# Visual-AI/SCD

Hardware: AMD Instinct MI355X
Metric: images/sec end-to-end (encode+sim+k-means) on 224^2 synth, 21k vocab (higher is better)
Workload: dtype f16; 1 GPU; ImageNet-100 unsupervised (BASELINE configs[1]): CLIP ViT-B/16 encode + V=21000 vocab + SSKM k=100 (10 restarts x 10 iters) + vote loop; cluster=SSKM, images_per_gpu=126976, vocab=21000, n_cluster=100, encode_batch=3990, weights=random-init (seeded), no checkpoint offline, parallelism=dp1

## Files before the change

### include/scd_hip.h

```cpp
#ifndef SCD_HIP_H
#define SCD_HIP_H
#include <stddef.h>
#include <stdint.h>

#ifdef __cplusplus
extern "C" {
#endif

typedef struct scd_ctx* scd_handle;
typedef struct scd_encoder scd_encoder;

enum scd_status { SCD_OK = 0, SCD_EINVAL = -1, SCD_EHIP = -2, SCD_ERCCL = -3, SCD_EINFEASIBLE = -4 };
enum scd_dtype { SCD_F32 = 0, SCD_F16 = 1 };
enum scd_sim_mode { SCD_SIM_RAW = 0, SCD_SIM_SOFTMAX = 1 };

int scd_version(void);
const char* scd_last_error(void);
int scd_create(int device, scd_handle* out);
int scd_destroy(scd_handle h);
int scd_trace_mark(scd_handle h, int end, void* stream);

int scd_l2norm_rows(scd_handle h, const void* x, int dtype, int64_t n, int d, void* out, void* stream);

size_t scd_sim_topk_ws_bytes(int64_t n, int d, int64_t v, int k);
// ... 175 lines not shown
int scd_comm_unique_id(void* id_out);
int scd_comm_init(scd_handle h, int rank, int world, const void* unique_id);
int scd_comm_destroy(scd_handle h);
int scd_allreduce_centroids(scd_handle h, double* packed, int64_t count, void* stream);
int scd_allgather_text(scd_handle h, const void* w_shard, int64_t shard_elems, void* w_full, void* stream);

typedef struct scd_encoder_desc {
    int kind;
    int width, layers, heads, mlp_dim;
    int tokens;
    int patch, image;
    int vocab;
    int out_dim;
    int act;
    float ln_eps;
    int registers;
} scd_encoder_desc;
int scd_encoder_create(scd_handle h, const scd_encoder_desc* desc, const void* const* weights, int n_weights,
                       scd_encoder** out);
int scd_encoder_destroy(scd_encoder* e);
size_t scd_encoder_ws_bytes(const scd_encoder* e, int batch);
int scd_encoder_timing(scd_encoder* e, int enable, double* ms_out, int* launches_out, double* flop_out);
int scd_vit_encode_image(scd_handle h, const scd_encoder* e, const void* pixels, int dtype, int batch, void* out,
                         int normalize, void* ws, size_t ws_bytes, void* stream);
int scd_clip_encode_text(scd_handle h, const scd_encoder* e, const int32_t* tokens, int batch, void* out,
                         int normalize, void* ws, size_t ws_bytes, void* stream);
int scd_clip_encode_text_len(scd_handle h, const scd_encoder* e, const int32_t* tokens, int batch, int ctx_len, void* out,
                             int normalize, void* ws, size_t ws_bytes, void* stream);
int scd_attention_f16(scd_handle h, const void* qkv, int batch, int T, int width, int heads, int causal, void* out, void* stream);
int scd_vit_assemble_f16(scd_handle h, const void* patch, const float* patch_bias, const float* cls, const float* pos,
                         const float* registers, int nreg, int batch, int T, int width, void* out, int64_t* stats, void* stream);
int scd_attention_single_query_f16(scd_handle h, const void* kv, const void* q, const int* qrow, int batch, int T, int width,
                                   int heads, int causal, void* out, void* stream);
int scd_gemm_f16(scd_handle h, const void* A, const void* W, const float* bias, const void* residual, void* C,
                 int64_t m, int n, int k, int act, void* stream);
int scd_gemm_ln_apply_f16(scd_handle h, const void* A, const void* Wf, const float* biasf, const float* colsum, const int64_t* stats_in,
                          float* rs, int64_t* zero_out, void* C, int64_t m, int n, int k, float eps, int act, void* stream);
int scd_gemm_res_stats_f16(scd_handle h, const void* A, const void* W, const float* bias, const void* residual, void* C,
                           int64_t* stats_out, int64_t m, int n, int k, int act, void* stream);
int scd_fold_ln_f16(scd_handle h, const void* W, const float* gamma, const float* beta, const float* bias, int n, int k, void* Wf,
                    float* colsum, float* biasf, void* stream);
int scd_gemm_img_f16(scd_handle h, const void* pixels, const void* W, void* C, int64_t m, int n, int batch, int image, void* stream);
int scd_layernorm_f16(scd_handle h, const void* x, const int* row_index, int64_t rows, int width, float eps, const float* gamma,
                      const float* beta, void* out, void* stream);

typedef struct scd_image_desc {
    int64_t src_off;
    int64_t tmp_off;
    int32_t w, h;
    int32_t plan_x;
    int32_t plan_y;
    int32_t row0, rows;
} scd_image_desc;
int scd_image_geometry(int w, int h, int size, int crop, int32_t* out6);
int scd_image_plan_axis(int in_size, int out_size, int off, int n, int32_t* first, int32_t* ntaps, int32_t* taps, int64_t taps_cap,
                        int64_t* n_taps_out);
int scd_image_batch_plan(const int32_t* wh, int batch, int size, int crop, scd_image_desc* descs, int32_t* plan, int64_t plan_cap,
                         int64_t* plan_len, int64_t* pixel_bytes, int64_t* ws_bytes);
int scd_image_preprocess(scd_handle h, const uint8_t* pixels, int64_t pixel_bytes, const scd_image_desc* descs, const int32_t* plan,
                         int64_t plan_len, int batch, int crop, const void* lut, void* out, void* ws, size_t ws_bytes, void* stream);

enum { SCD_JPEG_OK = 0, SCD_JPEG_NOT_JPEG = 1, SCD_JPEG_TRUNCATED = 2, SCD_JPEG_BAD_MARKER = 3, SCD_JPEG_PROGRESSIVE = 4, SCD_JPEG_ARITHMETIC = 5,
       SCD_JPEG_SOF = 6, SCD_JPEG_PRECISION = 7, SCD_JPEG_COMPONENTS = 8, SCD_JPEG_SAMPLING = 9, SCD_JPEG_COLOURSPACE = 10,
       SCD_JPEG_MULTISCAN = 11, SCD_JPEG_MISSING_TABLE = 12, SCD_JPEG_BAD_TABLE = 13, SCD_JPEG_CHROMA_WIDTH = 14, SCD_JPEG_DNL = 15 };
enum { SCD_JPEG_EHUFF = 1, SCD_JPEG_EINDEX = 2, SCD_JPEG_EEOF = 3, SCD_JPEG_EMARKER = 4, SCD_JPEG_ERANGE = 5, SCD_JPEG_EDESC = 6 };
typedef struct scd_jpeg_info {
// ... 33 lines not shown
```

### scd_amd/_lib.py

```python
import ctypes as C
import os
import threading

_HERE = os.path.dirname(os.path.abspath(__file__))
_LIB_PATH = os.environ.get("SCD_HIP_LIB") or os.path.join(_HERE, "lib", "libscd_hip.so")

SCD_OK, SCD_EINVAL, SCD_EHIP, SCD_ERCCL, SCD_EINFEASIBLE = 0, -1, -2, -3, -4
SCD_F32, SCD_F16 = 0, 1
SIM_RAW, SIM_SOFTMAX = 0, 1


class ScdError(RuntimeError):
    def __init__(self, code, msg):
        super().__init__("libscd_hip: %s (status %d)" % (msg, code))
        self.code = code


class EncoderDesc(C.Structure):
    _fields_ = [("kind", C.c_int), ("width", C.c_int), ("layers", C.c_int), ("heads", C.c_int), ("mlp_dim", C.c_int),
                ("tokens", C.c_int), ("patch", C.c_int), ("image", C.c_int), ("vocab", C.c_int), ("out_dim", C.c_int),
                ("act", C.c_int), ("ln_eps", C.c_float), ("registers", C.c_int)]


_vp, _i, _i64, _sz, _f = C.c_void_p, C.c_int, C.c_int64, C.c_size_t, C.c_float
# ... 87 lines not shown
    "scd_link_components_ws_bytes": (_sz, [_i64]),
    "scd_link_components": (_i, [_vp, _i64, _vp, _vp, _i64, _vp, _vp, _vp, _sz, _vp]),
    "scd_segment_mean_unit": (_i, [_vp, _vp, _i64, _vp, _vp, _i, _i, _vp, _vp, _vp]),
    "scd_knn_ws_bytes": (_sz, [_i64, _i64, _i, _i]),
    "scd_knn_slots": (_i, []),
    "scd_knn": (_i, [_vp, _vp, _i64, _vp, _i64, _i, _i, _i64, _vp, _vp, _vp, _vp, _sz, _vp]),
    "scd_knn_vote": (_i, [_vp, _vp, _vp, _i64, _i, _i, _vp, _i64, _i, C.c_double, _vp, _vp, _vp]),
    "scd_munkres": (_i, [_vp, _i, _i, _vp, C.POINTER(_i)]),
    "scd_munkres_sparse": (_i, [_i, _i64, _vp, _vp, _vp, _vp, C.POINTER(_i)]),
    "scd_transport_solve": (_i, [_vp, _i64, _i, _i, _i, _vp, C.POINTER(_i64)]),
    "scd_transport_solve_batch": (_i, [_vp, _i64, _i, _i, _i, _i, _vp, _vp, _i]),
    "scd_comm_unique_id_bytes": (_sz, []),
    "scd_comm_unique_id": (_i, [_vp]),
    "scd_comm_init": (_i, [_vp, _i, _i, _vp]),
    "scd_comm_destroy": (_i, [_vp]),
    "scd_allreduce_centroids": (_i, [_vp, _vp, _i64, _vp]),
    "scd_allgather_text": (_i, [_vp, _vp, _i64, _vp, _vp]),
    "scd_encoder_create": (_i, [_vp, C.POINTER(EncoderDesc), C.POINTER(_vp), _i, C.POINTER(_vp)]),
    "scd_encoder_destroy": (_i, [_vp]),
    "scd_encoder_ws_bytes": (_sz, [_vp, _i]),
    "scd_encoder_timing": (_i, [_vp, _i, C.POINTER(C.c_double), C.POINTER(_i), C.POINTER(C.c_double)]),
    "scd_vit_encode_image": (_i, [_vp, _vp, _vp, _i, _i, _vp, _i, _vp, _sz, _vp]),
    "scd_clip_encode_text": (_i, [_vp, _vp, _vp, _i, _vp, _i, _vp, _sz, _vp]),
    "scd_clip_encode_text_len": (_i, [_vp, _vp, _vp, _i, _i, _vp, _i, _vp, _sz, _vp]),
    "scd_gemm_f16": (_i, [_vp, _vp, _vp, _vp, _vp, _vp, _i64, _i, _i, _i, _vp]),
    "scd_gemm_ln_apply_f16": (_i, [_vp, _vp, _vp, _vp, _vp, _vp, _vp, _vp, _vp, _i64, _i, _i, _f, _i, _vp]),
    "scd_gemm_res_stats_f16": (_i, [_vp, _vp, _vp, _vp, _vp, _vp, _vp, _i64, _i, _i, _i, _vp]),
    "scd_fold_ln_f16": (_i, [_vp, _vp, _vp, _vp, _vp, _i, _i, _vp, _vp, _vp, _vp]),
    "scd_gemm_img_f16": (_i, [_vp, _vp, _vp, _vp, _i64, _i, _i, _i, _vp]),
    "scd_layernorm_f16": (_i, [_vp, _vp, _vp, _i64, _i, _f, _vp, _vp, _vp, _vp]),
    "scd_attention_f16": (_i, [_vp, _vp, _i, _i, _i, _i, _i, _vp, _vp]),
    "scd_vit_assemble_f16": (_i, [_vp, _vp, _vp, _vp, _vp, _vp, _i, _i, _i, _i, _vp, _vp, _vp]),
    "scd_attention_single_query_f16": (_i, [_vp, _vp, _vp, _vp, _i, _i, _i, _i, _i, _vp, _vp]),
    "scd_image_geometry": (_i, [_i, _i, _i, _i, _vp]),
    "scd_image_plan_axis": (_i, [_i, _i, _i, _i, _vp, _vp, _vp, _i64, _vp]),
    "scd_image_batch_plan": (_i, [_vp, _i, _i, _i, _vp, _vp, _i64, _vp, _vp, _vp]),
    "scd_image_preprocess": (_i, [_vp, _vp, _i64, _vp, _vp, _i64, _i, _i, _vp, _vp, _vp, _sz, _vp]),
    "scd_jpeg_parse": (_i, [_vp, _i64, _vp, _vp, _i64]),
    "scd_jpeg_batch_plan": (_i, [_vp, _vp, _vp, _i, _vp, _vp, _i64, _vp, _vp, _vp]),
    "scd_jpeg_decode": (_i, [_vp, _vp, _i64, _vp, _vp, _i64, _i, _vp, _i64, _vp, _vp, _sz, _vp]),
    "scd_jpeg_decode_host": (_i, [_vp, _i64, _vp, _i64, _vp]),
}

IMAGE_DESC_FIELDS = [("src_off", "<i8"), ("tmp_off", "<i8"), ("w", "<i4"), ("h", "<i4"), ("plan_x", "<i4"), ("plan_y", "<i4"),
                     ("row0", "<i4"), ("rows", "<i4")]

JPEG_INFO_FIELDS = [(k, "<i4") for k in ("reason", "w", "h", "ncomp", "hs", "vs", "restart_interval", "file_len", "scan_off", "scan_end",
                                          "has_eoi", "n_restarts")] + [(k, "<i4", (3,)) for k in ("qt_off", "qt_prec", "dc_off", "ac_off")]
JPEG_DESC_FIELDS = [("data_off", "<i8"), ("out_off", "<i8"), ("plane_off", "<i8")] + \
                   [(k, "<i4") for k in ("data_len", "scan_off", "scan_end", "has_eoi", "w", "h", "ncomp", "hs", "vs", "restart_interval")] + \
                   [(k, "<i4", (3,)) for k in ("qt", "dc", "ac")] + [("pad_", "<i4")]

_lock = threading.Lock()
_lib = None


def lib_path():
    return _LIB_PATH


def load():
    global _lib
    with _lock:
        if _lib is not None:
            return _lib
        if not os.path.exists(_LIB_PATH):
# ... 66 lines not shown
```

### scd_amd/csrc/encoder.hip

```cpp
#include "common.h"
#include "gemm.h"
#include <vector>
#include <stdlib.h>

struct scd_encoder {
    scd_encoder_desc d;
    std::vector<const void*> w;
    bool timing = false;
    std::vector<std::pair<hipEvent_t, hipEvent_t>> ev;
    double timed_flop = 0.0;
    struct Folded { const half_t *wq, *w1; const float *csq, *bq, *cs1, *b1; };
    std::vector<Folded> folded;
    void* folded_mem = nullptr;
    int kp = 0;
    half_t* wpatch_pad = nullptr;
};

enum { W_PATCH = 0, W_PATCH_B = 1, W_CLS = 2, W_POS = 3, W_LNPRE_W = 4, W_LNPRE_B = 5, W_LNPOST_W = 6, W_LNPOST_B = 7,
       W_PROJ = 8, W_LAYER0 = 9, W_PER_LAYER = 12 };
static inline int w_registers(const scd_encoder_desc& d) { return W_LAYER0 + W_PER_LAYER * d.layers; }
enum { L_LN1_W = 0, L_LN1_B, L_QKV_W, L_QKV_B, L_PROJ_W, L_PROJ_B, L_LN2_W, L_LN2_B, L_FC1_W, L_FC1_B, L_FC2_W, L_FC2_B };

__device__ __forceinline__ void stats_acc(const half4& o, float* st1, float* st2) {
#pragma unroll
    for (int j = 0; j < 4; ++j) {
        const float f = (float)o[j];
        *st1 += f;
        *st2 = fmaf(f, f, *st2);
    }
}
__device__ __forceinline__ void stats_store(float s1, float s2, long long* stats, long long r, int lane) {
    s1 = wave_sum_f32(s1);
    s2 = wave_sum_f32(s2);
    if (lane == 0) {
        stats[2 * r] = __float2ll_rn(s1 * 16777216.f);
        stats[2 * r + 1] = __float2ll_rn(s2 * 1048576.f);
    }
}
template <int MAXG>
__device__ __forceinline__ void ln_row(const float (&v)[MAXG][4], int groups, int width, float eps, const float* g,
                                       const float* b, half_t* out, int lane, float* st1 = nullptr, float* st2 = nullptr) {
    float s = 0.f;
#pragma unroll
    for (int i = 0; i < MAXG; ++i)
        if (i < groups) s += v[i][0] + v[i][1] + v[i][2] + v[i][3];
    const float mean = wave_sum_f32(s) / (float)width;
    float q = 0.f;
#pragma unroll
    for (int i = 0; i < MAXG; ++i)
// ... 854 lines not shown
#pragma unroll
    for (int e = 0; e < 8; ++e) o8[e] = 0.f;
    for (int key = ks; key < nkeys; key += 8) {
        const half8 v8 = *(const half8*)(vbase + (size_t)key * ldk + 8 * dc);
        const float pk = ps[wv][key];
#pragma unroll
        for (int e = 0; e < 8; ++e) o8[e] = fmaf(pk, (float)v8[e], o8[e]);
    }
    half8 o;
#pragma unroll
    for (int e = 0; e < 8; ++e) {
        float v = o8[e];
        v += __shfl_xor(v, 8, 64);
        v += __shfl_xor(v, 16, 64);
        v += __shfl_xor(v, 32, 64);
        o[e] = (half_t)(v * inv);
    }
    if (ks == 0) *(half8*)(out + (size_t)img * width + head * 64 + 8 * dc) = o;
}

__global__ void __launch_bounds__(256) gather2_rows_kernel(const half_t* __restrict__ a, const half_t* __restrict__ b,
                                                           const int* __restrict__ rows, int n, int width,
                                                           half_t* __restrict__ dst_a, half_t* __restrict__ dst_b) {
    const int lane = threadIdx.x & 63;
    const int i = blockIdx.x * 4 + (threadIdx.x >> 6);
    if (i >= n) return;
    const size_t src = (size_t)rows[i] * width, dst = (size_t)i * width;
    for (int c = lane * 8; c < width; c += 512) {
        *(half8*)(dst_a + dst + c) = *(const half8*)(a + src + c);
        *(half8*)(dst_b + dst + c) = *(const half8*)(b + src + c);
    }
}

struct EncPad {
    int batch, bh;
    int tokens;
    long long rows, prows;
};
static inline EncPad make_pad(const scd_encoder_desc& d, int batch, int tokens = 0) {
    EncPad p;
    p.batch = batch;
    p.tokens = tokens > 0 ? tokens : d.tokens;
    p.bh = (batch + 255) / 256 * 256;
    p.rows = ((long long)batch * p.tokens + 255) / 256 * 256;
    p.prows = ((long long)batch * (p.tokens - 1 - d.registers) + 255) / 256 * 256;
    return p;
}

struct EncWs {
    half_t *x, *y, *qkv, *h, *cls, *outp;
    int* rows;
    long long *stats_a, *stats_b;
    half_t *xsel, *ysel, *hsel;
    long long* stats_sel;
    float* rs;
    size_t total;
};
static EncWs carve(const scd_encoder_desc& d, const EncPad& pad, char* base) {
    EncWs w;
    const size_t rows = (size_t)pad.rows;
    const int bp = pad.bh;
    size_t off = 0;
    auto take = [&](size_t bytes) { char* p = base ? base + off : nullptr; off += scd_align(bytes); return p; };
    w.x = (half_t*)take(rows * d.width * 2);
    w.y = (half_t*)take(rows * d.width * 2);
    w.qkv = (half_t*)take(rows * 3 * d.width * 2);
    w.h = (half_t*)take(rows * d.mlp_dim * 2);
    w.cls = (half_t*)take((size_t)bp * d.width * 2);
    w.outp = (half_t*)take((size_t)bp * (d.out_dim > 0 ? d.out_dim : d.width) * 2);
    w.rows = (int*)take((size_t)bp * 4);
    w.stats_a = (long long*)take(rows * 16);
    w.stats_b = (long long*)take(rows * 16);
    w.xsel = (half_t*)take((size_t)bp * d.width * 2);
    w.ysel = (half_t*)take((size_t)bp * d.width * 2);
    w.hsel = (half_t*)take((size_t)bp * d.mlp_dim * 2);
    w.stats_sel = (long long*)take((size_t)bp * 16);
    w.rs = (float*)take(rows * 8);
    w.total = off + 256;
    return w;
}

extern "C" int scd_encoder_create(scd_handle h, const scd_encoder_desc* desc, const void* const* weights, int n_weights,
                                  scd_encoder** out) {
    SCD_DEVICE_ENTRY(h, "scd_encoder_create");
    SCD_REQUIRE(h && desc && weights && out, "scd_encoder_create: null argument");
    const scd_encoder_desc& d = *desc;
    SCD_REQUIRE(d.kind >= 0 && d.kind <= 2, "scd_encoder_create: bad kind %d", d.kind);
    SCD_REQUIRE(d.width % 256 == 0 && d.width <= 1024 && d.width == d.heads * 64, "scd_encoder_create: width %d / heads %d (head_dim must be 64)", d.width, d.heads);
    SCD_REQUIRE(d.mlp_dim % 128 == 0 && d.layers > 0, "scd_encoder_create: bad mlp_dim/layers");
    SCD_REQUIRE(d.out_dim == 0 || d.out_dim % 128 == 0, "scd_encoder_create: out_dim %d must be a multiple of 128", d.out_dim);
    SCD_REQUIRE(d.registers >= 0 && (d.registers == 0 || d.kind == 2),
                "scd_encoder_create: registers = %d: register tokens exist for kind 2 (DINO-style ViT) only, got kind %d", d.registers, d.kind);
    const int n_expected = W_LAYER0 + W_PER_LAYER * d.layers + (d.registers > 0 ? 1 : 0);
    SCD_REQUIRE(n_weights == n_expected, "scd_encoder_create: expected %d weight pointers, got %d", n_expected, n_weights);
    if (d.kind == 1) {
        SCD_REQUIRE(d.tokens == 77 && d.vocab > 0, "scd_encoder_create: text tower expects 77 tokens");
        SCD_REQUIRE(weights[W_PATCH] && weights[W_POS] && weights[W_LNPOST_W] && weights[W_LNPOST_B] && weights[W_PROJ] && d.out_dim > 0,
                    "scd_encoder_create: text tower weight missing");
    } else {
        SCD_REQUIRE(d.patch > 0 && d.image % d.patch == 0 && scd_cdiv(3 * d.patch * d.patch, 64) * 64 <= 3 * d.width,
                    "scd_encoder_create: bad patch/image");
        const int np = (d.image / d.patch) * (d.image / d.patch);
        SCD_REQUIRE(d.tokens == np + 1 + d.registers && (d.tokens == 197 || (d.tokens >= 257 && d.tokens <= 288)),
                    "scd_encoder_create: visual tower expects (image/patch)^2 + 1 + registers = 197 or 257..288 tokens, got %d "
                    "(%d patches, %d registers)", d.tokens, np, d.registers);
        SCD_REQUIRE(d.registers == 0 || weights[w_registers(d)], "scd_encoder_create: registers = %d but the register rows are null", d.registers);
        SCD_REQUIRE(weights[W_PATCH] && weights[W_CLS] && weights[W_POS] && weights[W_LNPOST_W] && weights[W_LNPOST_B],
                    "scd_encoder_create: visual tower weight missing");
        SCD_REQUIRE((d.out_dim > 0) == (weights[W_PROJ] != nullptr), "scd_encoder_create: projection / out_dim mismatch");
    }
// ... 5 lines not shown
    e->w.assign(weights, weights + n_weights);
    if (d.kind != 1 && (3 * d.patch * d.patch) % 64 != 0) {
        const int kk = 3 * d.patch * d.patch;
        e->kp = (int)scd_cdiv(kk, 64) * 64;
        const long long n = (long long)d.width * e->kp;
        if (hipMalloc(&e->wpatch_pad, (size_t)n * 2) != hipSuccess) {
            delete e;
            SCD_REQUIRE(false, "scd_encoder_create: out of device memory for the padded patch weight");
        }
        pad_cols_kernel<<<(unsigned)scd_cdiv(n, 256), 256>>>((const half_t*)weights[W_PATCH], d.width, kk, e->kp, e->wpatch_pad);
        SCD_HIP(hipDeviceSynchronize());
    }
    if (d.width % 256 == 0 && d.mlp_dim % 256 == 0) {
        const size_t wq = (size_t)3 * d.width * d.width * 2, w1 = (size_t)d.mlp_dim * d.width * 2;
        const size_t vq = scd_align((size_t)3 * d.width * 4), v1 = scd_align((size_t)d.mlp_dim * 4);
        const size_t per_layer = scd_align(wq) + scd_align(w1) + 2 * vq + 2 * v1;
        SCD_HIP(hipMalloc(&e->folded_mem, per_layer * d.layers));
        char* base = (char*)e->folded_mem;
        for (int l = 0; l < d.layers; ++l) {
            const void* const* lw = &e->w[W_LAYER0 + l * W_PER_LAYER];
            char* p = base + per_layer * l;
            half_t* fwq = (half_t*)p; p += scd_align(wq);
            half_t* fw1 = (half_t*)p; p += scd_align(w1);
            float* csq = (float*)p; p += vq;
            float* bq = (float*)p; p += vq;
            float* cs1 = (float*)p; p += v1;
            float* b1 = (float*)p;
            fold_ln_kernel<<<(3 * d.width + 3) / 4, 256>>>((const half_t*)lw[L_QKV_W], (const float*)lw[L_LN1_W], (const float*)lw[L_LN1_B],
                                                           (const float*)lw[L_QKV_B], 3 * d.width, d.width, fwq, csq, bq);
            fold_ln_kernel<<<(d.mlp_dim + 3) / 4, 256>>>((const half_t*)lw[L_FC1_W], (const float*)lw[L_LN2_W], (const float*)lw[L_LN2_B],
                                                         (const float*)lw[L_FC1_B], d.mlp_dim, d.width, fw1, cs1, b1);
            e->folded.push_back({fwq, fw1, csq, bq, cs1, b1});
        }
        SCD_HIP(hipDeviceSynchronize());
    }
    *out = e;
    return SCD_OK;
}

extern "C" int scd_encoder_destroy(scd_encoder* e) {
    if (e && e->folded_mem) hipFree(e->folded_mem);
    if (e && e->wpatch_pad) hipFree(e->wpatch_pad);
    delete e;
    return SCD_OK;
}

extern "C" int scd_encoder_timing(scd_encoder* e, int enable, double* ms_out, int* launches_out, double* flop_out) {
    SCD_REQUIRE(e, "scd_encoder_timing: null encoder");
    double ms = 0.0;
    for (auto& pr : e->ev) {
        SCD_HIP(hipEventSynchronize(pr.second));
        float t = 0.f;
        SCD_HIP(hipEventElapsedTime(&t, pr.first, pr.second));
        ms += t;
        hipEventDestroy(pr.first);
        hipEventDestroy(pr.second);
    }
    if (ms_out) *ms_out = ms;
    if (launches_out) *launches_out = (int)e->ev.size();
    if (flop_out) *flop_out = e->timed_flop;
    e->ev.clear();
    e->timed_flop = 0.0;
    e->timing = enable != 0;
    return SCD_OK;
}

extern "C" size_t scd_encoder_ws_bytes(const scd_encoder* e, int batch) {
    if (!e || batch <= 0) return 0;
    return carve(e->d, make_pad(e->d, batch), nullptr).total;
}

static int launch_attention(const half_t* qkv, half_t* out, int batch, int T, int width, int heads, int causal, hipStream_t st) {
    SCD_REQUIRE(batch > 0 && T > 0 && heads > 0 && width == heads * 64 && width <= 1024,
                "attention: batch %d, T %d, width %d / heads %d (head_dim must be 64, width <= 1024)", batch, T, width, heads);
    const int items = batch * heads;
// ... 17 lines not shown
        if (attn_short) attention_short_kernel<<<(items + 3) / 4, 256, 0, st>>>(qkv, out, T, width, heads, causal, items);
        else attention_kernel<1><<<items, 256, 0, st>>>(qkv, out, T, width, heads, causal, 0);
    }
    else if (T <= 64) attention_kernel<2><<<items, 256, 0, st>>>(qkv, out, T, width, heads, causal, 0);
    else if (T <= 96) attention_kernel<3><<<items, 256, 0, st>>>(qkv, out, T, width, heads, causal, 0);
    else SCD_REQUIRE(false, "attention: no kernel for %s T = %d (served: T <= 96, T = 197, non-causal 192 < T <= 224 with SCD_ATTN_PERSIST on, "
                            "non-causal 256 < T <= 288)",
                     causal ? "causal" : "non-causal", T);
    return SCD_OK;
}

static bool ln_fused(const scd_encoder* e, const EncPad& pad) {
    static const int ln_fuse_env = getenv("SCD_LN_FUSE") ? atoi(getenv("SCD_LN_FUSE")) : 1;
    return ln_fuse_env && !e->folded.empty() && pad.rows % 256 == 0;
}
static int run_blocks(const scd_encoder* e, const EncWs& w, const EncPad& pad, hipStream_t st, bool* selected_out) {
    const scd_encoder_desc& d = e->d;
    const long long rows = pad.rows;
    const int bp = pad.batch;
    const int act = d.act == 0 ? SCD_ACT_QUICKGELU : SCD_ACT_GELU;
    const int causal = d.kind == 1;
    const bool fuse = ln_fused(e, pad);
    static const int last_sel_env = getenv("SCD_LAST_SEL") ? atoi(getenv("SCD_LAST_SEL")) : 1;
    const bool last_sel = last_sel_env && d.mlp_dim % 256 == 0 && d.width % 256 == 0;
    *selected_out = last_sel;
    for (int l = 0; l < d.layers; ++l) {
        const void* const* lw = &e->w[W_LAYER0 + l * W_PER_LAYER];
        int rc;
        static const int last_q_env = getenv("SCD_LAST_Q") ? atoi(getenv("SCD_LAST_Q")) : 1;
        const bool last_q = last_sel && fuse && last_q_env && l == d.layers - 1 && d.width % 128 == 0 && pad.tokens <= 256;
        if (last_q) {
            const int bh = pad.bh;
            const size_t wk = (size_t)d.width * d.width;
            rc = scd_gemm_ln_finish(w.stats_a, rows, 1.0f / (float)d.width, d.ln_eps, w.rs, nullptr, st);
            if (rc) return rc;
            scd_gemm_ln lkv{w.stats_a, e->folded[l].csq + d.width, 1.0f / (float)d.width, d.ln_eps, nullptr, nullptr, w.rs};
            rc = scd_gemm_launch_ln(w.x, e->folded[l].wq + wk, e->folded[l].bq + d.width, nullptr, w.qkv, rows, 2 * d.width, d.width,
                                    SCD_ACT_NONE, &lkv, st);
            if (rc) return rc;
            gather_rows_stats_kernel<<<(unsigned)scd_cdiv(bh, 4), 256, 0, st>>>(w.x, w.stats_a, w.rows, bh, d.width, w.xsel, w.stats_sel);
            rc = scd_gemm_ln_finish(w.stats_sel, bh, 1.0f / (float)d.width, d.ln_eps, w.rs, nullptr, st);
            if (rc) return rc;
            scd_gemm_ln lq{w.stats_sel, e->folded[l].csq, 1.0f / (float)d.width, d.ln_eps, nullptr, nullptr, w.rs};
            rc = scd_gemm_launch_ln(w.xsel, e->folded[l].wq, e->folded[l].bq, nullptr, w.hsel, bh, d.width, d.width, SCD_ACT_NONE, &lq, st);
            if (rc) return rc;
            const int items = bp * d.heads;
            attention_single_query_kernel<<<(unsigned)scd_cdiv(items, 4), 256, 0, st>>>(w.qkv, w.hsel, w.rows, w.ysel, pad.tokens, d.width,
                                                                                         d.heads, items, causal);
            SCD_HIP(hipMemsetAsync(w.stats_sel, 0, (size_t)bh * 16, st));
            scd_gemm_ln lo{nullptr, nullptr, 0.f, 0.f, w.stats_sel, nullptr, nullptr};
            rc = scd_gemm_launch_ln(w.ysel, (const half_t*)lw[L_PROJ_W], (const float*)lw[L_PROJ_B], w.xsel, w.xsel, bh, d.width, d.width,
                                    SCD_ACT_NONE, &lo, st);
            if (rc) return rc;
            rc = scd_gemm_ln_finish(w.stats_sel, bh, 1.0f / (float)d.width, d.ln_eps, w.rs, nullptr, st);
            if (rc) return rc;
            scd_gemm_ln li{w.stats_sel, e->folded[l].cs1, 1.0f / (float)d.width, d.ln_eps, nullptr, nullptr, w.rs};
            rc = scd_gemm_launch_ln(w.xsel, e->folded[l].w1, e->folded[l].b1, nullptr, w.hsel, bh, d.mlp_dim, d.width, act, &li, st);
            if (rc) return rc;
            rc = scd_gemm_launch(w.hsel, (const half_t*)lw[L_FC2_W], (const float*)lw[L_FC2_B], w.xsel, w.xsel, bh, d.width, d.mlp_dim,
                                 SCD_ACT_NONE, st);
            if (rc) return rc;
            break;
        }
        if (fuse) {
            rc = scd_gemm_ln_finish(w.stats_a, rows, 1.0f / (float)d.width, d.ln_eps, w.rs, w.stats_b, st);
            if (rc) return rc;
            scd_gemm_ln ln{w.stats_a, e->folded[l].csq, 1.0f / (float)d.width, d.ln_eps, nullptr, w.stats_b, w.rs};
            rc = scd_gemm_launch_ln(w.x, e->folded[l].wq, e->folded[l].bq, nullptr, w.qkv, rows, 3 * d.width, d.width, SCD_ACT_NONE, &ln, st);
        } else {
            layernorm_kernel<<<(unsigned)scd_cdiv(rows, 4), 256, 0, st>>>(w.x, nullptr, rows, d.width, d.ln_eps, (const float*)lw[L_LN1_W],
                                                                           (const float*)lw[L_LN1_B], w.y);
            rc = scd_gemm_launch(w.y, (const half_t*)lw[L_QKV_W], (const float*)lw[L_QKV_B], nullptr, w.qkv, rows, 3 * d.width,
                                 d.width, SCD_ACT_NONE, st);
        }
        if (rc) return rc;
        rc = launch_attention(w.qkv, w.y, bp, pad.tokens, d.width, d.heads, causal, st);
        if (rc) return rc;
        if (last_sel && l == d.layers - 1) {
            const int bh = pad.bh;
            gather2_rows_kernel<<<(unsigned)scd_cdiv(bh, 4), 256, 0, st>>>(w.y, w.x, w.rows, bh, d.width, w.ysel, w.xsel);
            if (fuse) {
// ... 184 lines not shown
    SCD_LAUNCH_CHECK();
    return SCD_OK;
}

extern "C" int scd_attention_single_query_f16(scd_handle h, const void* kv, const void* q, const int* qrow, int batch, int T, int width,
                                              int heads, int causal, void* out, void* stream) {
    SCD_DEVICE_ENTRY(h, "scd_attention_single_query_f16");
    SCD_REQUIRE(kv && q && out && (qrow || !causal), "scd_attention_single_query_f16: null argument");
    SCD_REQUIRE(batch > 0 && T > 0 && T <= 256 && heads > 0 && width == heads * 64 && width <= 1024,
                "scd_attention_single_query_f16: batch %d, T %d (at most 256), width %d / heads %d (head_dim must be 64, width <= 1024)",
                batch, T, width, heads);
    const int items = batch * heads;
    attention_single_query_kernel<<<(unsigned)scd_cdiv(items, 4), 256, 0, (hipStream_t)stream>>>((const half_t*)kv, (const half_t*)q, qrow,
                                                                                                 (half_t*)out, T, width, heads, items, causal != 0);
    SCD_LAUNCH_CHECK();
    return SCD_OK;
}

extern "C" int scd_vit_assemble_f16(scd_handle h, const void* patch, const float* patch_bias, const float* cls, const float* pos,
                                    const float* registers, int nreg, int batch, int T, int width, void* out, int64_t* stats, void* stream) {
    SCD_DEVICE_ENTRY(h, "scd_vit_assemble_f16");
    SCD_REQUIRE(patch && cls && pos && out, "scd_vit_assemble_f16: null argument");
    SCD_REQUIRE(batch > 0 && width > 0 && width % 256 == 0 && width <= 1024, "scd_vit_assemble_f16: batch %d, width %d (a multiple of 256, at most 1024)",
                batch, width);
    SCD_REQUIRE(nreg >= 0 && T >= 2 + nreg && (nreg == 0 || registers), "scd_vit_assemble_f16: T = %d needs 1 + nreg = %d + at least one patch row%s",
                T, nreg, nreg > 0 && !registers ? " (registers is null)" : "");
    const long long rows = ((long long)batch * T + 255) / 256 * 256;
    launch_assemble((const half_t*)patch, patch_bias, cls, pos, registers, nreg, rows, batch, T, width, nullptr, nullptr, 0.f, (half_t*)out,
                    (long long*)stats, (hipStream_t)stream);
    SCD_LAUNCH_CHECK();
    return SCD_OK;
}

extern "C" int scd_gemm_ln_apply_f16(scd_handle h, const void* A, const void* Wf, const float* biasf, const float* colsum,
                                     const int64_t* stats_in, float* rs, int64_t* zero_out, void* C, int64_t m, int n, int k, float eps,
                                     int act, void* stream) {
    SCD_DEVICE_ENTRY(h, "scd_gemm_ln_apply_f16");
    SCD_REQUIRE(A && Wf && biasf && colsum && stats_in && rs && C, "scd_gemm_ln_apply_f16: null argument");
    SCD_REQUIRE(m > 0 && m % 256 == 0 && n > 0 && n % 256 == 0 && k > 0 && k % 64 == 0 && m < (1ll << 31),
                "scd_gemm_ln_apply_f16: shape m=%lld n=%d k=%d must be multiples of 256/256/64", (long long)m, n, k);
    SCD_REQUIRE(C != A, "scd_gemm_ln_apply_f16: C must not alias A");
    SCD_REQUIRE(act == SCD_ACT_NONE || act == SCD_ACT_QUICKGELU || act == SCD_ACT_GELU, "scd_gemm_ln_apply_f16: bad activation %d", act);
    hipStream_t st = (hipStream_t)stream;
    int rc = scd_gemm_ln_finish((const long long*)stats_in, m, 1.0f / (float)k, eps, rs, (long long*)zero_out, st);
    if (rc) return rc;
    scd_gemm_ln ln{(const long long*)stats_in, colsum, 1.0f / (float)k, eps, nullptr, (long long*)zero_out, rs};
    return scd_gemm_launch_ln((const half_t*)A, (const half_t*)Wf, biasf, nullptr, (half_t*)C, m, n, k, act, &ln, st);
}

extern "C" int scd_gemm_res_stats_f16(scd_handle h, const void* A, const void* W, const float* bias, const void* residual, void* C,
                                      int64_t* stats_out, int64_t m, int n, int k, int act, void* stream) {
    SCD_DEVICE_ENTRY(h, "scd_gemm_res_stats_f16");
    SCD_REQUIRE(stats_out, "scd_gemm_res_stats_f16: null statistics buffer");
    SCD_REQUIRE(n > 0 && k > 0, "scd_gemm_res_stats_f16: bad shape n=%d k=%d", n, k);
    scd_gemm_ln ln{nullptr, nullptr, 0.f, 0.f, (long long*)stats_out, nullptr, nullptr};
    return scd_gemm_launch_ln((const half_t*)A, (const half_t*)W, bias, (const half_t*)residual, (half_t*)C, m, n, k, act, &ln,
                              (hipStream_t)stream);
}

extern "C" int scd_fold_ln_f16(scd_handle h, const void* W, const float* gamma, const float* beta, const float* bias, int n, int k,
                               void* Wf, float* colsum, float* biasf, void* stream) {
    SCD_DEVICE_ENTRY(h, "scd_fold_ln_f16");
    SCD_REQUIRE(W && gamma && beta && bias && Wf && colsum && biasf && Wf != W, "scd_fold_ln_f16: null or aliased argument");
    SCD_REQUIRE(n > 0 && k > 0, "scd_fold_ln_f16: bad shape n=%d k=%d", n, k);
    fold_ln_kernel<<<(n + 3) / 4, 256, 0, (hipStream_t)stream>>>((const half_t*)W, gamma, beta, bias, n, k, (half_t*)Wf, colsum, biasf);
    SCD_LAUNCH_CHECK();
// ... 22 lines not shown
```

### scd_amd/ops.py

```python
import ctypes as C
import os

import numpy as np
import weakref

import torch

from . import _lib
from ._lib import check, ptr, SCD_F16, SCD_F32, SIM_RAW, SIM_SOFTMAX

_L = _lib.load
_dev = [None]


def _need_cuda(*ts):
    for t in ts:
        if t is not None and not t.is_cuda:
            raise _lib.ScdError(_lib.SCD_EINVAL, "tensor must live on the HIP device (got %s)" % t.device)
    for t in ts:
        if t is not None:
            _dev[0] = t.device.index
            break


# ... 1023 lines not shown

def vit_assemble_f16(patch, patch_bias, cls, pos, registers, batch, T, stats=False):
    _need_cuda(patch)
    _f16c(patch)
    width = patch.shape[1]
    nreg = 0 if registers is None else registers.shape[0]
    np_ = T - 1 - nreg
    _f32c(cls, pos, *[t for t in (patch_bias, registers) if t is not None])
    assert patch.shape == (batch * np_, width) and cls.shape == (width,) and pos.shape == (1 + np_, width)
    assert patch_bias is None or patch_bias.shape == (width,)
    assert registers is None or (nreg > 0 and registers.shape == (nreg, width))
    rows = (batch * T + 255) // 256 * 256
    out = torch.empty((rows, width), dtype=torch.float16, device=patch.device)
    st = torch.empty((rows, 2), dtype=torch.int64, device=patch.device) if stats else None
    check(_L().scd_vit_assemble_f16(handle(), ptr(patch), ptr(patch_bias), ptr(cls), ptr(pos), ptr(registers), nreg, int(batch), int(T),
                                    width, ptr(out), ptr(st), stream_ptr()))
    return (out, st) if stats else out


def attention_single_query_f16(kv, q, qrow, T, heads, causal=False):
    _need_cuda(kv, q)
    batch, width = q.shape
    assert kv.dtype == torch.float16 and q.dtype == torch.float16 and kv.is_contiguous() and q.is_contiguous()
    assert kv.shape == (batch * T, 2 * width)
    if qrow is not None:
        qrow = qrow.to(device=q.device, dtype=torch.int32).contiguous()
        assert qrow.shape == (batch,)
    out = torch.empty((batch, width), dtype=torch.float16, device=q.device)
    check(_L().scd_attention_single_query_f16(handle(), ptr(kv), ptr(q), ptr(qrow), int(batch), int(T), width, int(heads),
                                              1 if causal else 0, ptr(out), stream_ptr()))
    return out


class Encoder:

    def __init__(self, desc, weights):
        self.desc = desc
        self.weights = weights
        _need_cuda(next(w for w in weights if w is not None))
        arr = (C.c_void_p * len(weights))(*[None if w is None else w.data_ptr() for w in weights])
        enc = C.c_void_p()
        d = _lib.EncoderDesc(**desc)
        check(_L().scd_encoder_create(handle(), C.byref(d), arr, len(weights), C.byref(enc)))
        self._enc = enc
        self._ws = None
        self.out_dim = desc["out_dim"] if desc["out_dim"] > 0 else desc["width"]
        self.device = next(w for w in weights if w is not None).device

    def __del__(self):
        try:
            if getattr(self, "_enc", None):
                _L().scd_encoder_destroy(self._enc)
        except Exception:
            pass

    def timing(self, enable):
        ms, n, fl = C.c_double(0), C.c_int(0), C.c_double(0)
        check(_L().scd_encoder_timing(self._enc, 1 if enable else 0, C.byref(ms), C.byref(n), C.byref(fl)))
        return ms.value, n.value, fl.value

    def _workspace(self, batch):
        nb = _L().scd_encoder_ws_bytes(self._enc, batch)
        if self._ws is None or self._ws.numel() < nb:
            self._ws = _ws(nb, self.device)
        return self._ws, nb

# ... 29 lines not shown
```

Measured before the change: 30730 images/sec.

## Compute last-layer CLS attention directly from x, skipping the full K/V GEMM

For the final layer, where only the CLS query matters, the full K/V projection over all tokens is no longer run. Instead the per-head query is folded through the transposed key weight, giving one vector per head. A new fused kernel then scores the normalized x rows against those vectors with an online softmax and accumulates a per-head weighted sum of x. The value projection is applied afterwards to only batch*heads rows. This trades a large rows x 2W x W GEMM for small GEMMs plus one streaming pass over x, at the cost of extra workspace, a transposed weight copy and a more complex kernel.

```diff
diff --git a/include/scd_hip.h b/include/scd_hip.h
--- a/include/scd_hip.h
+++ b/include/scd_hip.h
@@ -231,6 +231,8 @@
                          const float* registers, int nreg, int batch, int T, int width, void* out, int64_t* stats, void* stream);
 int scd_attention_single_query_f16(scd_handle h, const void* kv, const void* q, const int* qrow, int batch, int T, int width,
                                    int heads, int causal, void* out, void* stream);
+int scd_cls_attention_x_f16(scd_handle h, const void* x, const float* rs, const void* u, int batch, int T, int width, int heads,
+                            void* out, void* stream);
 int scd_gemm_f16(scd_handle h, const void* A, const void* W, const float* bias, const void* residual, void* C,
                  int64_t m, int n, int k, int act, void* stream);
 int scd_gemm_ln_apply_f16(scd_handle h, const void* A, const void* Wf, const float* biasf, const float* colsum, const int64_t* stats_in,
diff --git a/scd_amd/_lib.py b/scd_amd/_lib.py
--- a/scd_amd/_lib.py
+++ b/scd_amd/_lib.py
@@ -143,6 +143,7 @@
     "scd_attention_f16": (_i, [_vp, _vp, _i, _i, _i, _i, _i, _vp, _vp]),
     "scd_vit_assemble_f16": (_i, [_vp, _vp, _vp, _vp, _vp, _vp, _i, _i, _i, _i, _vp, _vp, _vp]),
     "scd_attention_single_query_f16": (_i, [_vp, _vp, _vp, _vp, _i, _i, _i, _i, _i, _vp, _vp]),
+    "scd_cls_attention_x_f16": (_i, [_vp, _vp, _vp, _vp, _i, _i, _i, _i, _vp, _vp]),
     "scd_image_geometry": (_i, [_i, _i, _i, _i, _vp]),
     "scd_image_plan_axis": (_i, [_i, _i, _i, _i, _vp, _vp, _vp, _i64, _vp]),
     "scd_image_batch_plan": (_i, [_vp, _i, _i, _i, _vp, _vp, _i64, _vp, _vp, _vp]),
diff --git a/scd_amd/csrc/encoder.hip b/scd_amd/csrc/encoder.hip
--- a/scd_amd/csrc/encoder.hip
+++ b/scd_amd/csrc/encoder.hip
@@ -14,7 +14,9 @@
     void* folded_mem = nullptr;
     int kp = 0;
     half_t* wpatch_pad = nullptr;
+    half_t* wkt_last = nullptr;
 };
+static inline bool last_x_shape(const scd_encoder_desc& d) { return d.kind != 1 && d.tokens <= 256 && d.width % 256 == 0; }
 
 enum { W_PATCH = 0, W_PATCH_B = 1, W_CLS = 2, W_POS = 3, W_LNPRE_W = 4, W_LNPRE_B = 5, W_LNPOST_W = 6, W_LNPOST_B = 7,
        W_PROJ = 8, W_LAYER0 = 9, W_PER_LAYER = 12 };
@@ -935,6 +937,212 @@
     }
 }
 
+
+__global__ void __launch_bounds__(256) transpose_sq_kernel(const half_t* __restrict__ w, int n, half_t* __restrict__ wt) {
+    const long long e = (long long)blockIdx.x * 256 + threadIdx.x;
+    if (e >= (long long)n * n) return;
+    const int r = (int)(e / n), c = (int)(e % n);
+    wt[e] = w[(size_t)c * n + r];
+}
+
+__global__ void __launch_bounds__(256) expand_q_heads_kernel(const half_t* __restrict__ q, int batch, long long rows_out, int width,
+                                                             int heads, half_t* __restrict__ qx) {
+    const int lane = threadIdx.x & 63;
+    const long long row = (long long)blockIdx.x * 4 + (threadIdx.x >> 6);
+    if (row >= rows_out) return;
+    const long long b = row / heads;
+    const int h = (int)(row - b * heads);
+    for (int c = lane * 8; c < width; c += 512) {
+        half8 v = {0, 0, 0, 0, 0, 0, 0, 0};
+        if (b < batch && (c >> 6) == h) v = *(const half8*)(q + (size_t)b * width + c);
+        *(half8*)(qx + (size_t)row * width + c) = v;
+    }
+}
+
+__global__ void __launch_bounds__(256) pick_head_cols_kernel(const half_t* __restrict__ o, int batch, int n, int width, int heads,
+                                                             half_t* __restrict__ dst) {
+    const int lane = threadIdx.x & 63;
+    const int b = blockIdx.x * 4 + (threadIdx.x >> 6);
+    if (b >= n) return;
+    for (int c = lane * 8; c < width; c += 512) {
+        half8 v = {0, 0, 0, 0, 0, 0, 0, 0};
+        if (b < batch) v = *(const half8*)(o + ((size_t)b * heads + (c >> 6)) * width + c);
+        *(half8*)(dst + (size_t)b * width + c) = v;
+    }
+}
+
+typedef _Float16 half2v __attribute__((ext_vector_type(2)));
+typedef float f32x2 __attribute__((ext_vector_type(2)));
+
+template <int NI>
+__global__ void __launch_bounds__(256, NI <= 3 ? 2 : 1) cls_attention_x_kernel(const half_t* __restrict__ x, const float2* __restrict__ rs,
+                                                              const half_t* __restrict__ u, half_t* __restrict__ out, int T) {
+    constexpr int W = 256 * NI, H = 4 * NI, R = NI <= 3 ? 4 : 2, RH = R * H;
+    static_assert((H / 2) * W <= 2 * RH * 128, "the hand-over of slot 1 reuses the score partials' LDS");
+    __shared__ __attribute__((aligned(16))) float red[2][RH][128];
+    __shared__ __attribute__((aligned(16))) float pbuf[2][RH];
+    __shared__ __attribute__((aligned(16))) float abuf[2][H];
+    __shared__ float stt[2][H][3];
+    const int tid = threadIdx.x, slot = tid >> 7, ts = tid & 127;
+    const size_t row0 = (size_t)blockIdx.x * T;
+    const half_t* xb = x + row0 * W + 2 * ts;
+    const float2* rsb = rs + row0;
+    half2v u2[H][NI];
+#pragma unroll
+    for (int h = 0; h < H; ++h)
+#pragma unroll
+        for (int i = 0; i < NI; ++i) u2[h][i] = *(const half2v*)(u + ((size_t)blockIdx.x * H + h) * W + 256 * i + 2 * ts);
+    f32x2 acc[H][NI];
+#pragma unroll
+    for (int h = 0; h < H; ++h)
+#pragma unroll
+        for (int i = 0; i < NI; ++i) acc[h][i] = f32x2{0.f, 0.f};
+    const int rq = (ts >> 1) & (R - 1), hq = ts >> (R == 4 ? 3 : 2);
+    float mraw = -INFINITY, mxs = -INFINITY, offe = 0.f, lsum = 0.f;
+    const int nchunks = (T + R - 1) / R, iters = (nchunks + 1) / 2;
+    half2v xn[R][NI];
+    float2 rn[R];
+    auto load_chunk = [&](int chunk) {
+#pragma unroll
+        for (int r = 0; r < R; ++r) {
+            const int t = chunk * R + r < T ? chunk * R + r : T - 1;
+            rn[r] = rsb[t];
+#pragma unroll
+            for (int i = 0; i < NI; ++i) xn[r][i] = *(const half2v*)(xb + (size_t)t * W + 256 * i);
+        }
+    };
+    load_chunk(slot);
+    for (int it = 0; it < iters; ++it) {
+        const int chunk = 2 * it + slot;
+        f32x2 z[R][NI];
+#pragma unroll
+        for (int r = 0; r < R; ++r)
+#pragma unroll
+            for (int i = 0; i < NI; ++i) {
+                z[r][i].x = fmaf((float)xn[r][i].x, rn[r].x, rn[r].y);
+                z[r][i].y = fmaf((float)xn[r][i].y, rn[r].x, rn[r].y);
+            }
+        load_chunk(chunk + 2);
+#pragma unroll
+        for (int h = 0; h < H; ++h)
+#pragma unroll
+            for (int r = 0; r < R; ++r) {
+                float d = 0.f;
+#pragma unroll
+                for (int i = 0; i < NI; ++i) {
+                    d = fmaf((float)u2[h][i].x, z[r][i].x, d);
+                    d = fmaf((float)u2[h][i].y, z[r][i].y, d);
+                }
+                red[slot][h * R + r][ts] = d;
+            }
+        __syncthreads();
+        if (ts < 2 * RH) {
+            const float* base = &red[slot][ts >> 1][64 * (ts & 1)];
+            float s = 0.f;
+#pragma unroll
+            for (int k = 0; k < 16; ++k) {
+                const f32x4 q4 = *(const f32x4*)(base + 4 * ((k + ts) & 15));
+                s += (q4[0] + q4[1]) + (q4[2] + q4[3]);
+            }
+            s += __shfl_xor(s, 1, 64);
+            if (chunk * R + rq >= T) s = -INFINITY;
+            float cm = fmaxf(s, __shfl_xor(s, 2, 64));
+            if (R == 4) cm = fmaxf(cm, __shfl_xor(cm, 4, 64));
+            const float mn = fmaxf(mraw, cm);
+            const bool none = mn == -INFINITY;
+            const float cs = 0.125f * 1.4426950408889634f;
+            const float mxn = mn * cs;
+            const bool large = max_offset_is_large(mn, cs, mxn);
+            const float offn = large && !none ? fmaf(mn, cs, -mxn) : 0.f;
+            const float pe = __builtin_amdgcn_exp2f(fmaf(s, cs, -mxn) - offn);
+            const float ae = __builtin_amdgcn_exp2f((mxs - mxn) + (offe - offn));
+            const float p = none ? 0.f : pe, alpha = none ? 1.f : ae;
+            float psum = p + __shfl_xor(p, 2, 64);
+            if (R == 4) psum += __shfl_xor(psum, 4, 64);
+            lsum = fmaf(lsum, alpha, psum);
+            mraw = mn;
+            mxs = mxn;
+            offe = offn;
+            if (!(ts & 1)) {
+                pbuf[slot][ts >> 1] = p;
+                if (rq == 0) abuf[slot][hq] = alpha;
+            }
+        }
+        __syncthreads();
+#pragma unroll
+        for (int g = 0; g < NI; ++g) {
+            const f32x4 a4 = *(const f32x4*)&abuf[slot][4 * g];
+#pragma unroll
+            for (int e = 0; e < 4; ++e)
+#pragma unroll
+                for (int i = 0; i < NI; ++i) acc[4 * g + e][i] *= a4[e];
+        }
+#pragma unroll
+        for (int v4 = 0; v4 < RH / 4; ++v4) {
+            const f32x4 p4 = *(const f32x4*)&pbuf[slot][4 * v4];
+#pragma unroll
+            for (int e = 0; e < 4; ++e) {
+                const int h = (4 * v4 + e) / R, r = (4 * v4 + e) % R;
+#pragma unroll
+                for (int i = 0; i < NI; ++i) acc[h][i] += p4[e] * z[r][i];
+            }
+        }
+    }
+    if (ts < 2 * RH && !(ts & 1) && rq == 0) {
+        stt[slot][hq][0] = mxs;
+        stt[slot][hq][1] = offe;
+        stt[slot][hq][2] = lsum;
+    }
+    float* xch = &red[0][0][0];
+#pragma unroll
+    for (int k = 0; k < 2; ++k) {
+        __syncthreads();
+        if (slot == 1) {
+#pragma unroll
+            for (int hh = 0; hh < H / 2; ++hh)
+#pragma unroll
+                for (int i = 0; i < NI; ++i) *(f32x2*)(xch + hh * W + 256 * i + 2 * ts) = acc[k * (H / 2) + hh][i];
+        }
+        __syncthreads();
+        if (slot == 0) {
+#pragma unroll
+            for (int hh = 0; hh < H / 2; ++hh) {
+                const int h = k * (H / 2) + hh;
+                const float m0 = stt[0][h][0], o0 = stt[0][h][1], l0 = stt[0][h][2];
+                const float m1 = stt[1][h][0], o1 = stt[1][h][1], l1 = stt[1][h][2];
+                const bool first = m0 > m1 || (m0 == m1 && o0 >= o1);
+                const float mn = first ? m0 : m1, on = first ? o0 : o1;
+                const float f0 = __builtin_amdgcn_exp2f((m0 - mn) + (o0 - on));
+                const float f1 = __builtin_amdgcn_exp2f((m1 - mn) + (o1 - on));
+                const float inv = __builtin_amdgcn_rcpf(fmaf(l0, f0, l1 * f1));
+#pragma unroll
+                for (int i = 0; i < NI; ++i) {
+                    const f32x2 o = *(const f32x2*)(xch + hh * W + 256 * i + 2 * ts);
+                    const f32x2 a = (acc[h][i] * f0 + o * f1) * inv;
+                    half2v r2;
+                    r2.x = (half_t)a.x;
+                    r2.y = (half_t)a.y;
+                    *(half2v*)(out + ((size_t)blockIdx.x * H + h) * W + 256 * i + 2 * ts) = r2;
+                }
+            }
+        }
+    }
+}
+
+static int launch_cls_attention_x(const half_t* x, const float* rs, const half_t* u, half_t* out, int batch, int T, int width, int heads,
+                                  hipStream_t st) {
+    SCD_REQUIRE(batch > 0 && T > 0 && T <= 256 && width % 256 == 0 && width <= 1024 && width == heads * 64,
+                "cls attention from x: batch %d, T %d (at most 256), width %d / heads %d (width a multiple of 256, at most 1024; head_dim 64)",
+                batch, T, width, heads);
+    switch (width / 256) {
+    case 1: cls_attention_x_kernel<1><<<batch, 256, 0, st>>>(x, (const float2*)rs, u, out, T); break;
+    case 2: cls_attention_x_kernel<2><<<batch, 256, 0, st>>>(x, (const float2*)rs, u, out, T); break;
+    case 3: cls_attention_x_kernel<3><<<batch, 256, 0, st>>>(x, (const float2*)rs, u, out, T); break;
+    default: cls_attention_x_kernel<4><<<batch, 256, 0, st>>>(x, (const float2*)rs, u, out, T); break;
+    }
+    return SCD_OK;
+}
+
 struct EncPad {
     int batch, bh;
     int tokens;
@@ -957,6 +1165,7 @@
     half_t *xsel, *ysel, *hsel;
     long long* stats_sel;
     float* rs;
+    half_t *hx_a, *hx_b;
     size_t total;
 };
 static EncWs carve(const scd_encoder_desc& d, const EncPad& pad, char* base) {
@@ -979,6 +1188,11 @@
     w.hsel = (half_t*)take((size_t)bp * d.mlp_dim * 2);
     w.stats_sel = (long long*)take((size_t)bp * 16);
     w.rs = (float*)take(rows * 8);
+    w.hx_a = w.hx_b = nullptr;
+    if (last_x_shape(d)) {
+        w.hx_a = (half_t*)take((size_t)d.heads * bp * d.width * 2);
+        w.hx_b = (half_t*)take((size_t)d.heads * bp * d.width * 2);
+    }
     w.total = off + 256;
     return w;
 }
@@ -1050,6 +1264,16 @@
                                                          (const float*)lw[L_FC1_B], d.mlp_dim, d.width, fw1, cs1, b1);
             e->folded.push_back({fwq, fw1, csq, bq, cs1, b1});
         }
+        if (last_x_shape(d)) {
+            const long long n = (long long)d.width * d.width;
+            if (hipMalloc(&e->wkt_last, (size_t)n * 2) != hipSuccess) {
+                hipFree(e->folded_mem);
+                if (e->wpatch_pad) hipFree(e->wpatch_pad);
+                delete e;
+                SCD_REQUIRE(false, "scd_encoder_create: out of device memory for the transposed key weight");
+            }
+            transpose_sq_kernel<<<(unsigned)scd_cdiv(n, 256), 256>>>(e->folded.back().wq + n, d.width, e->wkt_last);
+        }
         SCD_HIP(hipDeviceSynchronize());
     }
     *out = e;
@@ -1059,6 +1283,7 @@
 extern "C" int scd_encoder_destroy(scd_encoder* e) {
     if (e && e->folded_mem) hipFree(e->folded_mem);
     if (e && e->wpatch_pad) hipFree(e->wpatch_pad);
+    if (e && e->wkt_last) hipFree(e->wkt_last);
     delete e;
     return SCD_OK;
 }
@@ -1142,21 +1367,40 @@
         if (last_q) {
             const int bh = pad.bh;
             const size_t wk = (size_t)d.width * d.width;
-            rc = scd_gemm_ln_finish(w.stats_a, rows, 1.0f / (float)d.width, d.ln_eps, w.rs, nullptr, st);
-            if (rc) return rc;
-            scd_gemm_ln lkv{w.stats_a, e->folded[l].csq + d.width, 1.0f / (float)d.width, d.ln_eps, nullptr, nullptr, w.rs};
-            rc = scd_gemm_launch_ln(w.x, e->folded[l].wq + wk, e->folded[l].bq + d.width, nullptr, w.qkv, rows, 2 * d.width, d.width,
-                                    SCD_ACT_NONE, &lkv, st);
-            if (rc) return rc;
+            static const int last_x_env = getenv("SCD_LAST_X") ? atoi(getenv("SCD_LAST_X")) : 1;
+            const bool last_x = last_x_env && last_x_shape(d) && e->wkt_last && w.hx_a;
+            if (!last_x) {
+                rc = scd_gemm_ln_finish(w.stats_a, rows, 1.0f / (float)d.width, d.ln_eps, w.rs, nullptr, st);
+                if (rc) return rc;
+                scd_gemm_ln lkv{w.stats_a, e->folded[l].csq + d.width, 1.0f / (float)d.width, d.ln_eps, nullptr, nullptr, w.rs};
+                rc = scd_gemm_launch_ln(w.x, e->folded[l].wq + wk, e->folded[l].bq + d.width, nullptr, w.qkv, rows, 2 * d.width, d.width,
+                                        SCD_ACT_NONE, &lkv, st);
+                if (rc) return rc;
+            }
             gather_rows_stats_kernel<<<(unsigned)scd_cdiv(bh, 4), 256, 0, st>>>(w.x, w.stats_a, w.rows, bh, d.width, w.xsel, w.stats_sel);
             rc = scd_gemm_ln_finish(w.stats_sel, bh, 1.0f / (float)d.width, d.ln_eps, w.rs, nullptr, st);
             if (rc) return rc;
             scd_gemm_ln lq{w.stats_sel, e->folded[l].csq, 1.0f / (float)d.width, d.ln_eps, nullptr, nullptr, w.rs};
             rc = scd_gemm_launch_ln(w.xsel, e->folded[l].wq, e->folded[l].bq, nullptr, w.hsel, bh, d.width, d.width, SCD_ACT_NONE, &lq, st);
             if (rc) return rc;
-            const int items = bp * d.heads;
-            attention_single_query_kernel<<<(unsigned)scd_cdiv(items, 4), 256, 0, st>>>(w.qkv, w.hsel, w.rows, w.ysel, pad.tokens, d.width,
-                                                                                         d.heads, items, causal);
+            if (last_x) {
+                const long long hrows = (long long)d.heads * bh;
+                rc = scd_gemm_ln_finish(w.stats_a, rows, 1.0f / (float)d.width, d.ln_eps, w.rs, nullptr, st);
+                if (rc) return rc;
+                expand_q_heads_kernel<<<(unsigned)scd_cdiv(hrows, 4), 256, 0, st>>>(w.hsel, bp, hrows, d.width, d.heads, w.hx_a);
+                rc = scd_gemm_launch(w.hx_a, e->wkt_last, nullptr, nullptr, w.hx_b, hrows, d.width, d.width, SCD_ACT_NONE, st);
+                if (rc) return rc;
+                rc = launch_cls_attention_x(w.x, w.rs, w.hx_b, w.hx_a, bp, pad.tokens, d.width, d.heads, st);
+                if (rc) return rc;
+                rc = scd_gemm_launch(w.hx_a, e->folded[l].wq + 2 * wk, e->folded[l].bq + 2 * d.width, nullptr, w.hx_b, hrows, d.width,
+                                     d.width, SCD_ACT_NONE, st);
+                if (rc) return rc;
+                pick_head_cols_kernel<<<(unsigned)scd_cdiv(bh, 4), 256, 0, st>>>(w.hx_b, bp, bh, d.width, d.heads, w.ysel);
+            } else {
+                const int items = bp * d.heads;
+                attention_single_query_kernel<<<(unsigned)scd_cdiv(items, 4), 256, 0, st>>>(w.qkv, w.hsel, w.rows, w.ysel, pad.tokens, d.width,
+                                                                                             d.heads, items, causal);
+            }
             SCD_HIP(hipMemsetAsync(w.stats_sel, 0, (size_t)bh * 16, st));
             scd_gemm_ln lo{nullptr, nullptr, 0.f, 0.f, w.stats_sel, nullptr, nullptr};
             rc = scd_gemm_launch_ln(w.ysel, (const half_t*)lw[L_PROJ_W], (const float*)lw[L_PROJ_B], w.xsel, w.xsel, bh, d.width, d.width,
@@ -1407,6 +1651,16 @@
     return SCD_OK;
 }
 
+extern "C" int scd_cls_attention_x_f16(scd_handle h, const void* x, const float* rs, const void* u, int batch, int T, int width, int heads,
+                                       void* out, void* stream) {
+    SCD_DEVICE_ENTRY(h, "scd_cls_attention_x_f16");
+    SCD_REQUIRE(x && rs && u && out && out != u, "scd_cls_attention_x_f16: null or aliased argument");
+    const int rc = launch_cls_attention_x((const half_t*)x, rs, (const half_t*)u, (half_t*)out, batch, T, width, heads, (hipStream_t)stream);
+    if (rc) return rc;
+    SCD_LAUNCH_CHECK();
+    return SCD_OK;
+}
+
 extern "C" int scd_gemm_ln_apply_f16(scd_handle h, const void* A, const void* Wf, const float* biasf, const float* colsum,
                                      const int64_t* stats_in, float* rs, int64_t* zero_out, void* C, int64_t m, int n, int k, float eps,
                                      int act, void* stream) {
diff --git a/scd_amd/ops.py b/scd_amd/ops.py
--- a/scd_amd/ops.py
+++ b/scd_amd/ops.py
@@ -1079,6 +1079,18 @@
     return out
 
 
+def cls_attention_x_f16(x, rs, u, T, heads):
+    _need_cuda(x, rs, u)
+    width = x.shape[1]
+    batch = u.shape[0] // heads
+    assert x.dtype == torch.float16 and u.dtype == torch.float16 and rs.dtype == torch.float32
+    assert x.is_contiguous() and rs.is_contiguous() and u.is_contiguous()
+    assert x.shape == (batch * T, width) and rs.shape == (batch * T, 2) and u.shape == (batch * heads, width)
+    out = torch.empty((batch * heads, width), dtype=torch.float16, device=x.device)
+    check(_L().scd_cls_attention_x_f16(handle(), ptr(x), ptr(rs), ptr(u), int(batch), int(T), width, int(heads), ptr(out), stream_ptr()))
+    return out
+
+
 class Encoder:
 
     def __init__(self, desc, weights):
```

Result: no change. 31020 images/sec, median of 6 (+1.0%).
